# mennowitteveen/PySnpTools

Hardware: AMD Instinct MI355X
Metric: SNPs/sec standardized (500k×1M) + GRM GF/s at 1/2/4/8 GPUs (higher is better)
Workload: dtype f32; 1 GPU; decode+Unit standardize of the 500000 iid x 1000000 SNP matrix (packed BED resident in HBM, SnpGen MAF curve, 1% missing), SNPs split into 1 contiguous shard(s), block 2048 SNPs, f32 F-order block buffer with a 500000-float column pitch; n_iid=500000, n_sid=1000000, n_sid_per_gpu=1000000, block=2048, block_buffer_ld=500000, parallelism=snp-shard x1, process_group=none

## Files before the change

pysnptools_amd/csrc/api.hip:

```cpp
#include <fcntl.h>
#include <immintrin.h>
#include <sys/mman.h>
#include <sys/stat.h>
#include <unistd.h>

#include <algorithm>
#include <atomic>
#include <cmath>
#include <cstdlib>
#include <mutex>
#include <thread>
#include <vector>

#include "snpmi_internal.hpp"

#include <type_traits>

namespace snpmi {

static thread_local std::string g_last_error;
void set_last_error(const std::string& msg) { g_last_error = msg; }

static std::mutex g_dev_mutex;
static std::vector<Device*> g_devices;
// ... 1585 lines not shown

using namespace snpmi;

extern "C" {

const char* snpmi_last_error(void) { return g_last_error.c_str(); }
int snpmi_version(void) { return 1; }

int snpmi_device_count(int* count) {
    return guarded([&] {
        SNPMI_REQUIRE(count != nullptr, SNPMI_E_ARG, "count is NULL");
        *count = num_devices();
        (void)hipGetLastError();
    });
}

int snpmi_set_device(int dev) {
    return guarded([&] {
        SNPMI_REQUIRE(dev >= 0 && dev < num_devices(), SNPMI_E_ARG, "device index out of range");
        g_cur_dev = dev;
        (void)device();
    });
}

int snpmi_get_device(int* dev) {
    return guarded([&] {
        SNPMI_REQUIRE(dev != nullptr, SNPMI_E_ARG, "dev is NULL");
        *dev = g_cur_dev < 0 ? default_device() : g_cur_dev;
    });
}

int snpmi_release_cache(void) {
    return guarded([&] {
        std::lock_guard<std::recursive_mutex> lk(g_call_mutex);
        std::lock_guard<std::mutex> lk2(g_dev_mutex);
        for (Device* d : g_devices)
            if (d) {
                SNPMI_HIP(hipSetDevice(d->id));
                SNPMI_HIP(hipStreamSynchronize(d->stream));
                d->release();
            }
        release_pinned();
    });
}

int snpmi_device_info(int dev, char* name, size_t name_len, uint64_t* total_mem, int* cu_count) {
    return guarded([&] {
        hipDeviceProp_t p;
        SNPMI_HIP(hipGetDeviceProperties(&p, dev));
        if (name && name_len) {
            std::strncpy(name, p.gcnArchName, name_len - 1);
            name[name_len - 1] = 0;
        }
        if (total_mem) *total_mem = p.totalGlobalMem;
        if (cu_count) *cu_count = p.multiProcessorCount;
    });
}

int snpmi_device_ids(int dev, uint8_t* uuid16, int* pci, int* clock_khz) {
    return guarded([&] {
        hipDeviceProp_t p;
        SNPMI_HIP(hipGetDeviceProperties(&p, dev));
        if (uuid16) std::memcpy(uuid16, p.uuid.bytes, 16);
        if (pci) {
            pci[0] = p.pciDomainID;
            pci[1] = p.pciBusID;
            pci[2] = p.pciDeviceID;
        }
        if (clock_khz) *clock_khz = p.clockRate;
    });
}

struct Hook {
    const char* name;
    int* value;
    enum Kind { ANY, BOOL, CLAMP0, RANGE, LIST, READ_ONLY } kind;
    int lo, hi;
    std::vector<int> list;
    const char* what;
};
static const std::vector<Hook>& hooks() {
    static const std::vector<Hook> table = {
        {"decode", &g_variant_decode, Hook::ANY, 0, 0, {}, nullptr},
        {"std", &g_variant_std, Hook::ANY, 0, 0, {}, nullptr},
        {"diag", &g_diag_exact, Hook::BOOL, 0, 0, {}, nullptr},
        {"extract", &g_variant_extract, Hook::ANY, 0, 0, {}, nullptr},
        {"syrk", &g_variant_syrk, Hook::LIST, 0, 0, {0, 5, 20, 36, 71}, "syrk variant: a shipped kernel (0, 5, 20, 36, 71)"},
        {"syrk_split", &g_variant_syrk_split, Hook::ANY, 0, 0, {}, nullptr},
        {"dense_chunk", &g_dense_chunk, Hook::CLAMP0, 0, 0, {}, nullptr},
        {"dense_codes", &g_dense_codes, Hook::ANY, 0, 0, {}, nullptr},
        {"seg", &g_seg_snps, Hook::CLAMP0, 0, 0, {}, nullptr},
        {"gather", &g_gather, Hook::ANY, 0, 0, {}, nullptr},
        {"h2", &g_h2_kernel, Hook::RANGE, 0, 1, {}, "h2 SYRK: 0 = k_syrk_h2, 1 = k_syrk_h2s"},
        {"crt", &g_crt_kernel, Hook::RANGE, 0, 2, {},
         "crt residue SYRK: 0 = k_syrk_i8r, 1 = k_syrk_i8w, 2 = k_syrk_i8w without its read order / wave priorities"},
        {"crt_block", &g_crt_block, Hook::RANGE, 0, 1, {}, "crt moduli: 0 = launch-wide R, 1 = per 256-block"},
        {"f64", &g_f64_mfma, Hook::RANGE, 0, 1, {}, "f64 GRM path: 0 = int8 residues + CRT, 1 = f64 MFMA"},
        {"overlap_groups", &g_last_groups, Hook::READ_ONLY, 0, 0, {}, nullptr},
        {"overlap_calls", &g_last_sum_calls, Hook::READ_ONLY, 0, 0, {}, nullptr},
        {"overlap_sig", &g_last_sum_sig31, Hook::READ_ONLY, 0, 0, {}, nullptr},
    };
    return table;
}
static const Hook& find_hook(const char* name) {
    for (const Hook& h : hooks())
        if (std::strcmp(name, h.name) == 0) return h;
    throw Error(SNPMI_E_ARG, std::string("unknown kernel ") + name);
}

int snpmi_set_kernel_variant(const char* kernel, int variant) {
    return guarded([&] {
        SNPMI_REQUIRE(kernel != nullptr, SNPMI_E_ARG, "kernel name is NULL");
        const Hook& h = find_hook(kernel);
        const bool ok = h.kind == Hook::RANGE  ? variant >= h.lo && variant <= h.hi
                        : h.kind == Hook::LIST ? std::find(h.list.begin(), h.list.end(), variant) != h.list.end()
                                               : h.kind != Hook::READ_ONLY;
        SNPMI_REQUIRE(ok, SNPMI_E_ARG,
                      h.what ? std::string(h.what) + " (got " + std::to_string(variant) + ")"
                             : std::string("unknown kernel ") + kernel);
        *h.value = h.kind == Hook::BOOL ? variant != 0 : h.kind == Hook::CLAMP0 ? std::max(variant, 0) : variant;
    });
}

int snpmi_get_kernel_variant(const char* kernel, int* variant) {
    return guarded([&] {
        SNPMI_REQUIRE(kernel != nullptr && variant != nullptr, SNPMI_E_ARG, "kernel name or output is NULL");
        *variant = *find_hook(kernel).value;
    });
}

int snpmi_bed_check(const char* path, uint64_t n_iid, uint64_t n_sid) {
    return guarded([&] {
        BedMap m;
        open_bed(m, path, n_iid, n_sid);
    });
}

#define SNPMI_BED_READ(SUFFIX, T)                                                                                  \
    int snpmi_bed_read_##SUFFIX(const char* path, uint64_t n_iid, uint64_t n_sid, int count_a1,                  \
                                const uint64_t* iid_idx, uint64_t n_out_iid, const uint64_t* sid_idx,             \
                                uint64_t n_out_sid, int order_c, T* out, int num_threads) {                       \
        return guarded([&] {                                                                                       \
            bed_read_impl<T>(path, n_iid, n_sid, count_a1, iid_idx, n_out_iid, sid_idx, n_out_sid, order_c,       \
                             SNPMI_STD_NONE, 0.0, 0.0, 0, (T*)nullptr, out, num_threads);                         \
        });                                                                                                        \
    }
SNPMI_BED_READ(f32, float)
SNPMI_BED_READ(f64, double)
SNPMI_BED_READ(i8, int8_t)

#define SNPMI_BED_READ_STD(SUFFIX, T)                                                                              \
    int snpmi_bed_read_standardize_##SUFFIX(const char* path, uint64_t n_iid, uint64_t n_sid, int count_a1,      \
                                            const uint64_t* iid_idx, uint64_t n_out_iid, const uint64_t* sid_idx, \
                                            uint64_t n_out_sid, int order_c, int std_kind, double a, double b,    \
                                            int use_stats, T* stats, T* out, int num_threads) {                   \
        return guarded([&] {                                                                                       \
            SNPMI_REQUIRE(std_kind == SNPMI_STD_NONE || stats != nullptr, SNPMI_E_ARG, "stats is NULL");          \
            bed_read_impl<T>(path, n_iid, n_sid, count_a1, iid_idx, n_out_iid, sid_idx, n_out_sid, order_c,       \
                             std_kind, a, b, use_stats, stats, out, num_threads);                                 \
        });                                                                                                        \
    }
SNPMI_BED_READ_STD(f32, float)
SNPMI_BED_READ_STD(f64, double)

#define SNPMI_BED_WRITE(SUFFIX, T)                                                                                 \
    int snpmi_bed_write_##SUFFIX(const char* path, const T* val, uint64_t n_iid, uint64_t n_sid, int order_c,    \
// ... 915 lines not shown
```

pysnptools_amd/csrc/kernels.hip:

```cpp
#include "snpmi_internal.hpp"

namespace snpmi {
namespace {

constexpr int kWave = 64;
constexpr int kBlock = 256;

__device__ __forceinline__ double stats_mean_std(double n, double s1, double s2, double* sd_out) {
    if (n == 0.0) {
        *sd_out = __builtin_nan("");
        return __builtin_nan("");
    }
    double m = s1 / n;
    double var = s2 / n - m * m;
    double sd = sqrt(var);
    if (!(sd > 0.0)) sd = __builtin_inf();
    *sd_out = sd;
    return m;
}

__device__ __forceinline__ double beta_weight(double mean, double a, double b) {
    double maf = mean / 2.0;
    if (maf > 0.5) maf = 1.0 - maf;
    if (!(maf >= 0.0 && maf <= 1.0)) return 0.0;
// ... 67 lines not shown
                count_word(v.w);
            };
            const uint64_t nfull = n / 64;
            constexpr uint64_t step = (uint64_t)W * kWave;
            uint64_t q = (uint64_t)sub * kWave + lane;
            for (; q + (U - 1) * step < nfull; q += U * step) {
                uint4 v[U];
#pragma unroll
                for (int u = 0; u < U; u++) v[u] = col[q + u * step];
#pragma unroll
                for (int u = 0; u < U; u++) count16(v[u]);
            }
            for (; q < nfull; q += step) count16(col[q]);
            if (q == nfull && n % 64) {
                const uint4 v = col[q];
                const uint32_t w4[4] = {v.x, v.y, v.z, v.w};
#pragma unroll
                for (int k = 0; k < 4; k++) {
                    const uint64_t ib = q * 64 + 16 * k;
                    const uint64_t valid_i = n > ib ? min<uint64_t>(n - ib, 16) : 0;
                    const uint32_t mk = valid_i >= 16 ? 0xffffffffu : ((1u << (2 * valid_i)) - 1u);
                    count_word(w4[k] & mk);
                }
            }
            c1 = clo - c3;
            c2 = chi - c3;
        }
        c1 = wave_sum_u32(c1);
        c2 = wave_sum_u32(c2);
        c3 = wave_sum_u32(c3);
        if constexpr (W > 1) {
            if (lane == 0) {
                red[wave][0] = c1;
                red[wave][1] = c2;
                red[wave][2] = c3;
            }
            __syncthreads();
            if (!valid || sub != 0) return;
#pragma unroll
            for (int w = 1; w < W; w++) {
                c1 += red[wave + w][0];
                c2 += red[wave + w][1];
                c3 += red[wave + w][2];
            }
        }
        uint64_t c0 = n - c1 - c2 - c3;
        uint64_t chi = count_a1 ? c0 : c3;
        double nobs = (double)(n - c1);
        mean = stats_mean_std(nobs, (double)(c2 + 2 * chi), (double)(c2 + 4 * chi), &sd);
        if (lane == 0) {
            stats[2 * s] = (T)mean;
            stats[2 * s + 1] = (T)sd;
        }
    }
    if (lane < 4) {
        double w = std_kind == SNPMI_STD_BETA ? beta_weight(mean, a, b) : 0.0;
        bool zero_col = std_kind == SNPMI_STD_BETA && use_stats && __builtin_isinf(sd);
        int v = code_value(lane, count_a1);
        double x;
        if (v < 0 || zero_col) x = 0.0;
        else if (std_kind == SNPMI_STD_BETA) x = ((double)v - mean) * w;
        else x = ((double)v - mean) / sd;
        lut[4 * s + lane] = (T)x;
    }
}

template <typename T>
__device__ __forceinline__ T sel4(T l0, T l1, T l2, T l3, uint32_t c) {
    const bool b0 = (c & 1u) != 0, b1 = (c & 2u) != 0;
    const T lo = b0 ? l1 : l0;
    const T hi = b0 ? l3 : l2;
    return b1 ? hi : lo;
}

typedef float f32x4_t __attribute__((ext_vector_type(4)));
typedef double f64x2_t __attribute__((ext_vector_type(2)));
typedef uint32_t u32x4_t __attribute__((ext_vector_type(4)));

template <typename V>
__device__ __forceinline__ void store_nt(V* p, const V& v) {
    __builtin_nontemporal_store(v, p);
}
template <typename T, int U>
__global__ __launch_bounds__(kBlock) void k_decode_f(const uint8_t* __restrict__ packed, uint64_t pitch, uint64_t n,
                                                     uint64_t m, const T* __restrict__ lut, T* __restrict__ out,
                                                     uint64_t ld) {
    const int lane = threadIdx.x & (kWave - 1);
    const uint64_t chunks = (n + 1023) / 1024;
    const uint64_t total = chunks * m;
    const uint64_t groups = (total + U - 1) / U;
    const uint64_t nwaves = (uint64_t)gridDim.x * (kBlock / kWave);
    const uint64_t lb = (blockIdx.x & 7) * (gridDim.x >> 3) + (blockIdx.x >> 3);
    for (uint64_t gi = lb * (kBlock / kWave) + threadIdx.x / kWave; gi < groups; gi += nwaves) {
        uint32_t w[U];
        uint64_t jv[U], cv[U];
        bool val[U];
#pragma unroll
        for (int u = 0; u < U; u++) {
            const uint64_t it = gi * U + u;
            const uint64_t j = it / chunks, c = it - j * chunks;
            jv[u] = j;
            cv[u] = c;
            val[u] = it < total;
            const bool ok = val[u] && (c * 1024 + 16 * (uint64_t)lane < n);
            w[u] = ok ? reinterpret_cast<const uint32_t*>(packed + j * pitch)[c * 64 + lane] : 0u;
        }
#pragma unroll
        for (int u = 0; u < U; u++) {
            if (!val[u]) continue;
            const uint64_t j = jv[u], i0 = cv[u] * 1024;
            const T l0 = lut[4 * j], l1 = lut[4 * j + 1], l2 = lut[4 * j + 2], l3 = lut[4 * j + 3];
            T* o = out + j * ld + i0;
            if constexpr (sizeof(T) == 4) {
#pragma unroll
                for (int r = 0; r < 4; r++) {
                    const uint32_t src = __shfl(w[u], r * 16 + (lane >> 2), kWave);
                    const uint32_t byte = (src >> (8 * (lane & 3))) & 0xffu;
                    const uint64_t i = i0 + r * 256 + 4 * lane;
                    f32x4_t v;
                    v.x = sel4(l0, l1, l2, l3, byte & 3u);
                    v.y = sel4(l0, l1, l2, l3, (byte >> 2) & 3u);
                    v.z = sel4(l0, l1, l2, l3, (byte >> 4) & 3u);
                    v.w = sel4(l0, l1, l2, l3, byte >> 6);
                    if (i + 4 <= n) {
                        store_nt(reinterpret_cast<f32x4_t*>(o + r * 256 + 4 * lane), v);
                    } else {
                        for (int t = 0; t < 4; t++)
                            if (i + t < n) o[r * 256 + 4 * lane + t] = v[t];
                    }
                }
            } else if constexpr (sizeof(T) == 8) {
#pragma unroll
                for (int r = 0; r < 8; r++) {
                    const uint32_t src = __shfl(w[u], r * 8 + (lane >> 3), kWave);
                    const uint32_t byte = (src >> (8 * ((lane >> 1) & 3))) & 0xffu;
                    const uint32_t sh = 4 * (lane & 1);
                    const uint64_t i = i0 + r * 128 + 2 * lane;
                    f64x2_t v;
                    v.x = sel4(l0, l1, l2, l3, (byte >> sh) & 3u);
                    v.y = sel4(l0, l1, l2, l3, (byte >> (sh + 2)) & 3u);
                    if (i + 2 <= n) {
                        store_nt(reinterpret_cast<f64x2_t*>(o + r * 128 + 2 * lane), v);
                    } else if (i < n) {
                        o[r * 128 + 2 * lane] = v.x;
                    }
                }
            } else {
                const uint32_t lw = (uint32_t)(uint8_t)l0 | ((uint32_t)(uint8_t)l1 << 8) |
                                    ((uint32_t)(uint8_t)l2 << 16) | ((uint32_t)(uint8_t)l3 << 24);
                u32x4_t q;
#pragma unroll
                for (int k = 0; k < 4; k++) {
                    const uint32_t bb = (w[u] >> (8 * k)) & 0xffu;
                    const uint32_t selb = (bb & 3u) | ((bb & 0xCu) << 6) | ((bb & 0x30u) << 12) | ((bb & 0xC0u) << 18);
                    q[k] = __builtin_amdgcn_perm(0u, lw, selb);
                }
                const uint64_t i = i0 + 16 * lane;
                if (i + 16 <= n) {
                    store_nt(reinterpret_cast<u32x4_t*>(o + 16 * lane), q);
                } else if (i < n) {
                    for (uint64_t t = 0; i + t < n; t++)
                        reinterpret_cast<uint8_t*>(o)[16 * lane + t] = (uint8_t)(q[t >> 2] >> (8 * (t & 3)));
                }
            }
        }
    }
}


template <int U>
__global__ __launch_bounds__(kBlock) void k_decode_std_col_f32(const uint8_t* __restrict__ packed, uint64_t pitch,
                                                               uint64_t n, int count_a1, int std_kind, double a,
                                                               double b, int use_stats, float* __restrict__ stats,
                                                               float* __restrict__ lut_out, float* __restrict__ out,
                                                               uint64_t ld) {
    __shared__ uint32_t red[3][kBlock / kWave];
    __shared__ float lutsh[4];
    const int lane = threadIdx.x & (kWave - 1), wave = threadIdx.x / kWave;
    const uint64_t j = blockIdx.x;
    const uint8_t* colp = packed + j * pitch;
    if (std_kind == SNPMI_STD_NONE) {
        if (threadIdx.x < 4) {
            int v = code_value(threadIdx.x, count_a1);
            lutsh[threadIdx.x] = v < 0 ? __builtin_nanf("") : (float)v;
        }
    } else {
        double mean = 0, sd = 0;
        if (!use_stats) {
            const uint4* col = reinterpret_cast<const uint4*>(colp);
            const uint64_t nq = (n + 63) / 64;
            uint32_t c1 = 0, c2 = 0, c3 = 0;
            for (uint64_t q0 = threadIdx.x; q0 < nq; q0 += kBlock * 4) {
                uint4 vv[4];
#pragma unroll
                for (int u = 0; u < 4; u++) {
                    const uint64_t q = q0 + (uint64_t)u * kBlock;
                    vv[u] = q < nq ? col[q] : make_uint4(0, 0, 0, 0);
                }
#pragma unroll
                for (int u = 0; u < 4; u++) {
                    const uint64_t q = q0 + (uint64_t)u * kBlock;
                    uint32_t w4[4] = {vv[u].x, vv[u].y, vv[u].z, vv[u].w};
#pragma unroll
                    for (int k = 0; k < 4; k++) {
                        uint32_t w = w4[k];
                        uint32_t lo = w & 0x55555555u, hi = (w >> 1) & 0x55555555u;
                        const uint64_t ib = q * 64 + 16 * k;
                        if (ib + 16 > n) {
                            const uint64_t valid = n > ib ? n - ib : 0;
                            const uint32_t mk = valid >= 16 ? 0xFFFFFFFFu : (((1u << (2 * valid)) - 1u) & 0x55555555u);
                            lo &= mk;
                            hi &= mk;
                        }
                        c3 += __popc(lo & hi);
                        c2 += __popc(hi & ~lo);
                        c1 += __popc(lo & ~hi);
                    }
                }
            }
            c1 = wave_sum_u32(c1);
            c2 = wave_sum_u32(c2);
            c3 = wave_sum_u32(c3);
            if (lane == 0) {
                red[0][wave] = c1;
                red[1][wave] = c2;
                red[2][wave] = c3;
            }
            __syncthreads();
            if (threadIdx.x == 0) {
                uint64_t t1 = 0, t2 = 0, t3 = 0;
                for (int q = 0; q < kBlock / kWave; q++) {
                    t1 += red[0][q];
                    t2 += red[1][q];
                    t3 += red[2][q];
                }
                const uint64_t c0 = n - t1 - t2 - t3, chi = count_a1 ? c0 : t3;
                mean = stats_mean_std((double)(n - t1), (double)(t2 + 2 * chi), (double)(t2 + 4 * chi), &sd);
                stats[2 * j] = (float)mean;
                stats[2 * j + 1] = (float)sd;
            }
        } else if (threadIdx.x == 0) {
            mean = (double)stats[2 * j];
            sd = (double)stats[2 * j + 1];
        }
        if (threadIdx.x == 0) {
            const double w = std_kind == SNPMI_STD_BETA ? beta_weight(mean, a, b) : 0.0;
            const bool zero_col = std_kind == SNPMI_STD_BETA && use_stats && __builtin_isinf(sd);
            for (int c = 0; c < 4; c++) {
// ... 1377 lines not shown
        c2 = wave_sum_u32(c2);
        c3 = wave_sum_u32(c3);
        if (lane == 0) {
            red[0][wave] = c1;
            red[1][wave] = c2;
            red[2][wave] = c3;
        }
    }
    __syncthreads();
    if (threadIdx.x == 0) {
        if (std_kind == SNPMI_STD_NONE) {
            for (int c = 0; c < 4; c++) {
                const int v = code_value(c, count_a1);
                lutsh[c] = v < 0 ? __builtin_nanf("") : (float)v;
            }
        } else {
            double mean, sd;
            if (count) {
                uint64_t t1 = 0, t2 = 0, t3 = 0;
                for (int q = 0; q < kLdsBlock / kWave; q++) {
                    t1 += red[0][q];
                    t2 += red[1][q];
                    t3 += red[2][q];
                }
                const uint64_t c0 = n - t1 - t2 - t3, chi = count_a1 ? c0 : t3;
                mean = stats_mean_std((double)(n - t1), (double)(t2 + 2 * chi), (double)(t2 + 4 * chi), &sd);
                stats[2 * j] = (float)mean;
                stats[2 * j + 1] = (float)sd;
            } else {
                mean = (double)stats[2 * j];
                sd = (double)stats[2 * j + 1];
            }
            const double w = std_kind == SNPMI_STD_BETA ? beta_weight(mean, a, b) : 0.0;
            const bool zero_col = std_kind == SNPMI_STD_BETA && use_stats && __builtin_isinf(sd);
            for (int c = 0; c < 4; c++) {
                const int v = code_value(c, count_a1);
                double x;
                if (v < 0 || zero_col) x = 0.0;
                else if (std_kind == SNPMI_STD_BETA) x = ((double)v - mean) * w;
                else x = ((double)v - mean) / sd;
                lutsh[c] = (float)x;
            }
        }
        for (int c = 0; c < 4; c++) lut_out[4 * j + c] = lutsh[c];
    }
    __syncthreads();
    const float l0 = lutsh[0], l1 = lutsh[1], l2 = lutsh[2], l3 = lutsh[3];
    const uint32_t* cw = reinterpret_cast<const uint32_t*>(col);
    float* o = out + j * ld;
    const uint64_t chunks = (n + 1023) / 1024;
    for (uint64_t c = wave; c < chunks; c += kLdsBlock / kWave) {
        const uint64_t i0 = c * 1024;
        const uint32_t wv = (i0 + 16 * (uint64_t)lane < n) ? cw[c * 64 + lane] : 0u;
#pragma unroll
        for (int r = 0; r < 4; r++) {
            const uint32_t srcw = __shfl(wv, r * 16 + (lane >> 2), kWave);
            const uint32_t byte = (srcw >> (8 * (lane & 3))) & 0xffu;
            const uint64_t i = i0 + r * 256 + 4 * lane;
            f32x4_t v;
            v.x = sel4(l0, l1, l2, l3, byte & 3u);
            v.y = sel4(l0, l1, l2, l3, (byte >> 2) & 3u);
            v.z = sel4(l0, l1, l2, l3, (byte >> 4) & 3u);
            v.w = sel4(l0, l1, l2, l3, byte >> 6);
            if (i + 4 <= n) {
                store_nt(reinterpret_cast<f32x4_t*>(o + i), v);
            } else {
                for (int t = 0; t < 4; t++)
                    if (i + t < n) o[i + t] = v[t];
            }
        }
    }
}

inline unsigned grid_for(uint64_t work, uint64_t per_block, unsigned cap = 65536) {
    uint64_t g = (work + per_block - 1) / per_block;
    if (g < 1) g = 1;
    if (g > cap) g = cap;
    return (unsigned)g;
}

}

int g_variant_decode = 0;
int g_diag_exact = 1;
int g_variant_std = 0;
int g_variant_extract = 0;

#define SNPMI_LAUNCH_CHECK() SNPMI_HIP(hipGetLastError())

void launch_snp_stats(const uint8_t* packed, uint64_t pitch, uint64_t n, uint64_t m, int count_a1, int std_kind,
                      double a, double b, int use_stats, int dtype, void* stats, void* lut, hipStream_t st) {
    if (m == 0) return;
    const bool wide = n >= 65536 && g_variant_decode != 6;
#define SNPMI_STATS(T, W, kind)                                                                                    \
    k_snp_stats<T, W><<<(unsigned)ceil_div(m, kBlock / kWave / W), kBlock, 0, st>>>(                               \
        packed, pitch, n, m, count_a1, kind, a, b, dtype == SNPMI_DT_I8 ? 0 : use_stats, (T*)stats, (T*)lut)
#define SNPMI_STATS_U(T, W, U, kind)                                                                               \
    k_snp_stats<T, W, U><<<(unsigned)ceil_div(m, kBlock / kWave / W), kBlock, 0, st>>>(                            \
        packed, pitch, n, m, count_a1, kind, a, b, dtype == SNPMI_DT_I8 ? 0 : use_stats, (T*)stats, (T*)lut)
    if (dtype == SNPMI_DT_F32) {
        if (wide && g_variant_decode == 7) SNPMI_STATS_U(float, 4, 4, std_kind);
        else if (wide && g_variant_decode == 9) SNPMI_STATS_U(float, 4, 16, std_kind);
        else if (wide && g_variant_decode == 8) SNPMI_STATS(float, 2, std_kind);
        else if (wide) SNPMI_STATS(float, 4, std_kind);
        else SNPMI_STATS(float, 1, std_kind);
    } else if (dtype == SNPMI_DT_F64) {
        if (wide) SNPMI_STATS(double, 4, std_kind);
        else SNPMI_STATS(double, 1, std_kind);
    } else {
        SNPMI_STATS(int8_t, 1, SNPMI_STD_NONE);
    }
#undef SNPMI_STATS
#undef SNPMI_STATS_U
    SNPMI_LAUNCH_CHECK();
}

void launch_decode(const uint8_t* packed, uint64_t pitch, uint64_t n, uint64_t m, const void* lut, int dtype,
                   int order_c, void* out, uint64_t ld, hipStream_t st) {
    if (m == 0 || n == 0) return;
    if (!order_c) {
        const uint64_t waves = ceil_div(ceil_div(n, 1024) * m, 4);
        const unsigned g = grid_for(waves, kBlock / kWave, 256 * 16 * 8);
        const unsigned g8 = (unsigned)round_up(g, 8);
        if (dtype == SNPMI_DT_F32)
            k_decode_f<float, 4><<<g8, kBlock, 0, st>>>(packed, pitch, n, m, (const float*)lut, (float*)out, ld);
        else if (dtype == SNPMI_DT_F64)
            k_decode_f<double, 4><<<g8, kBlock, 0, st>>>(packed, pitch, n, m, (const double*)lut, (double*)out, ld);
        else
            k_decode_f<int8_t, 4><<<g8, kBlock, 0, st>>>(packed, pitch, n, m, (const int8_t*)lut, (int8_t*)out, ld);
    } else {
        if (dtype != SNPMI_DT_I8 && g_variant_decode != 2 && ld % (16 / dtype_size(dtype)) == 0 &&
            reinterpret_cast<uintptr_t>(out) % 16 == 0 && pitch % 64 == 0) {
            const uint64_t V = 16 / dtype_size(dtype);
            const uint64_t waves = ceil_div(n, 256) * ceil_div(m, 64 * V);
            const unsigned g = grid_for(waves, kBlock / kWave, 256 * 16);
            if (dtype == SNPMI_DT_F32 && g_variant_decode == 3)
                k_decode_c_reg<float, true><<<g, kBlock, 0, st>>>(packed, pitch, n, m, (const float*)lut, (float*)out, ld);
            else if (dtype == SNPMI_DT_F32)
                k_decode_c_reg<float, false><<<g, kBlock, 0, st>>>(packed, pitch, n, m, (const float*)lut, (float*)out,
                                                                   ld);
            else
                k_decode_c_reg<double, false><<<g, kBlock, 0, st>>>(packed, pitch, n, m, (const double*)lut,
                                                                    (double*)out, ld);
            SNPMI_LAUNCH_CHECK();
            return;
        }
        const uint64_t tiles = ceil_div(n, 64) * ceil_div(m, 64);
        const unsigned g = grid_for(tiles, 1, 256 * 8);
        if (dtype == SNPMI_DT_F32)
            k_decode_c<float><<<g, kBlock, 0, st>>>(packed, pitch, n, m, (const float*)lut, (float*)out, ld);
        else if (dtype == SNPMI_DT_F64)
            k_decode_c<double><<<g, kBlock, 0, st>>>(packed, pitch, n, m, (const double*)lut, (double*)out, ld);
        else
            k_decode_c<int8_t><<<g, kBlock, 0, st>>>(packed, pitch, n, m, (const int8_t*)lut, (int8_t*)out, ld);
    }
    SNPMI_LAUNCH_CHECK();
}

void launch_decode_std_fused(const uint8_t* packed, uint64_t pitch, uint64_t n, uint64_t m, int count_a1,
                             int std_kind, double a, double b, int use_stats, void* stats, void* lut, void* out,
                             uint64_t ld, hipStream_t st) {
    if (m == 0 || n == 0) return;
    const uint64_t col_bytes = ceil_div(n, 64) * 16;
    if (g_variant_decode != 1 && col_bytes <= kLdsColMax) {
        SNPMI_HIP(hipFuncSetAttribute((const void*)k_decode_std_lds_f32, hipFuncAttributeMaxDynamicSharedMemorySize,
                                      (int)kLdsColMax));
        k_decode_std_lds_f32<<<(unsigned)m, kLdsBlock, col_bytes, st>>>(packed, pitch, n, count_a1, std_kind, a, b,
                                                                        use_stats, (float*)stats, (float*)lut,
                                                                        (float*)out, ld);
    } else {
        k_decode_std_col_f32<4><<<(unsigned)m, kBlock, 0, st>>>(packed, pitch, n, count_a1, std_kind, a, b, use_stats,
                                                                (float*)stats, (float*)lut, (float*)out, ld);
    }
    SNPMI_LAUNCH_CHECK();
}

uint64_t repack_plan_entries(uint64_t n_out) {
    const uint64_t n = std::max<uint64_t>(n_out, 1);
    return std::max(round_up(n, 16), ceil_div(n, kRepackChunk) * kRepackChunk / 2);
}
uint64_t repack_win_entries(uint64_t n_out) { return 3 * ceil_div(std::max<uint64_t>(n_out, 1), 4096) + 64; }

RepackPlan launch_repack_plan(const uint64_t* idx, uint64_t n_out, uint64_t n_src, uint32_t* plan, uint32_t* win,
                              hipStream_t st) {
    RepackPlan P;
    const uint64_t nq = ceil_div(ceil_div(n_src, 4), 16), n_pad = repack_plan_entries(n_out);
    if (n_out == 0) return P;
    const uint64_t chunk = g_variant_decode == 9 ? 16384 : g_variant_decode == 10 ? 4096 : kRepackChunk;
    const uint64_t nchunks = ceil_div(n_out, chunk);
    if (win != nullptr && nchunks > 1 && g_variant_decode != 8) {
        uint32_t* lohi = win + nchunks;
        std::vector<uint32_t> h(2 * nchunks);
        for (uint64_t c = 0; c < nchunks; c++) h[2 * c] = ~0u, h[2 * c + 1] = 0;
        SNPMI_HIP(hipMemcpyAsync(lohi, h.data(), h.size() * 4, hipMemcpyHostToDevice, st));
        k_repack_window<<<(unsigned)ceil_div(n_out, 2048), 256, 0, st>>>(idx, n_out, chunk, lohi);
        SNPMI_LAUNCH_CHECK();
        SNPMI_HIP(hipMemcpyAsync(h.data(), lohi, h.size() * 4, hipMemcpyDeviceToHost, st));
        SNPMI_HIP(hipStreamSynchronize(st));
        std::vector<uint32_t> lo4(nchunks);
        uint64_t w = 0;
        for (uint64_t c = 0; c < nchunks; c++) {
            lo4[c] = h[2 * c] >> 6;
            w = std::max<uint64_t>(w, (h[2 * c + 1] >> 6) - lo4[c] + 1);
        }
        const uint64_t budget = 40 * 1024 - 16;
        int K = 4 * w * 16 <= budget ? 4 : 2 * w * 16 <= budget ? 2 : w * 16 <= budget ? 1 : 0;
        if (g_variant_decode == 11 && K == 4) K = 2;
        if (K > 0 && 2 * w <= nq) {
            SNPMI_HIP(hipMemcpyAsync(win, lo4.data(), nchunks * 4, hipMemcpyHostToDevice, st));
            if (chunk == kRepackChunk && 4 * w < 4096 && g_variant_decode != 17) {
                const uint64_t n_all = nchunks * kRepackChunk;
                k_repack_plan16<<<grid_for(n_all, kBlock, 4096), kBlock, 0, st>>>(idx, n_out, n_all, w, win,
// ... 429 lines not shown
```

pysnptools_amd/csrc/snpmi_internal.hpp:

```cpp
#pragma once
#include <hip/hip_runtime.h>

#include <cstdint>
#include <cstring>
#include <functional>
#include <stdexcept>
#include <string>
#include <vector>

#include "../../include/snpmi.h"

namespace snpmi {

struct Error : std::runtime_error {
    int code;
    Error(int c, const std::string& m) : std::runtime_error(m), code(c) {}
};

void set_last_error(const std::string& msg);

#define SNPMI_HIP(expr)                                                                     \
    do {                                                                                    \
        hipError_t e_ = (expr);                                                             \
        if (e_ != hipSuccess)                                                               \
            throw ::snpmi::Error(SNPMI_E_HIP, std::string(#expr) + ": " + hipGetErrorString(e_)); \
    } while (0)

#define SNPMI_REQUIRE(cond, code, msg)                 \
    do {                                               \
        if (!(cond)) throw ::snpmi::Error(code, msg);  \
    } while (0)

template <class F>
int guarded(F&& body) {
    try {
        body();
        return SNPMI_OK;
    } catch (const Error& e) {
        set_last_error(e.what());
        return e.code;
    } catch (const std::bad_alloc&) {
        set_last_error("host allocation failed");
        return SNPMI_E_NOMEM;
    } catch (const std::exception& e) {
        set_last_error(e.what());
        return SNPMI_E_ARG;
    }
}

__device__ __forceinline__ uint64_t sgpr_u64(uint64_t v) {
    const uint32_t lo = (uint32_t)__builtin_amdgcn_readfirstlane((int)(uint32_t)v);
    const uint32_t hi = (uint32_t)__builtin_amdgcn_readfirstlane((int)(uint32_t)(v >> 32));
    return ((uint64_t)hi << 32) | (uint64_t)lo;
}
__device__ __forceinline__ void* sgpr_ptr(const void* p) {
    return reinterpret_cast<void*>(sgpr_u64(reinterpret_cast<uint64_t>(p)));
}

constexpr int kTile = 128;
inline uint64_t ceil_div(uint64_t a, uint64_t b) { return (a + b - 1) / b; }
inline uint64_t round_up(uint64_t a, uint64_t b) { return ceil_div(a, b) * b; }
inline uint64_t packed_pitch(uint64_t n_iid) { return round_up(ceil_div(n_iid, 4), 64); }
inline uint64_t n_tiles_1d(uint64_t n) { return ceil_div(n, kTile); }
inline uint64_t n_tiles_upper(uint64_t n) { uint64_t t = n_tiles_1d(n); return t * (t + 1) / 2; }
inline size_t dtype_size(int dt) { return dt == SNPMI_DT_F64 ? 8 : dt == SNPMI_DT_F32 ? 4 : 1; }

constexpr int kPieces = 4;
constexpr uint64_t kPieceBytes = 32ull << 20;

struct Device {
    int id = -1;
    hipStream_t stream = nullptr;
    hipStream_t copy = nullptr;
    hipStream_t aux = nullptr;
    int cu_count = 0;
    enum Slot { S_PACKED, S_PACKED2, S_IDX, S_IDX2, S_LUT, S_STATS, S_OUT, S_TILES, S_K, S_DENSE,
                S_DENSE2, S_RED, S_SESSION, S_PACKED_B, S_ZBLK, S_IDX32, S_LUT3, S_H2, S_OUT_B, S_STATS_B,
                S_WIN, S_DPACK, S_DLUT, S_CRTREC, S_SEG, S_STDFLAG, S_DIAG,
                S_RECT, S_RECT_A, S_RECT_B, S_RECT_IDX_A, S_RECT_IDX_B, S_RECT_PLAN_A, S_RECT_PLAN_B, S_RECT_WIN_A,
                S_RECT_WIN_B, S_RECT_PAIRS, S_NUM };
    void* buf[S_NUM] = {};
    hipEvent_t staged[2] = {};
    hipEvent_t consumed[2] = {};
    hipEvent_t produced[2] = {};
    hipEvent_t bounce[2] = {};
    hipEvent_t fence = nullptr;
    hipEvent_t piece[kPieces] = {};
    uint64_t piece_next = 0;
    size_t cap[S_NUM] = {};
    uint32_t* order_tab[2] = {};
    uint64_t order_nb[2] = {};
    void* part_tab = nullptr;
    uint64_t part_key[3] = {};
    void* get(Slot s, size_t bytes);
    void release();
};

Device& device();
hipStream_t stream();

void* pinned(int slot, size_t bytes);
void release_pinned();

extern int g_variant_decode;
extern int g_variant_std;
extern int g_variant_extract;
extern int g_dense_chunk;
extern int g_h2_kernel;
extern int g_seg_snps;
struct SegCtx {
    uint32_t snps = 0;
    uint32_t nslots = 0;
    uint32_t* flags = nullptr;
    float* scratch = nullptr;
};
constexpr uint32_t kSegSlots = 1024;
constexpr uint64_t kSegSlotFloats = 8 * 32 * 64 * 4;
SegCtx seg_ctx();
const uint32_t* packed_block_order(uint64_t nb);
uint64_t part_unit(uint64_t nb, int world);
void part_layout(uint64_t nb, int rank, int world, std::vector<uint32_t>& tab);
struct PartTables {
    const uint32_t* tab = nullptr;
    const int32_t* dslot = nullptr;
    const int32_t* lslot = nullptr;
};
PartTables part_tables(uint64_t nb, int rank, int world);
void launch_snp_stats(const uint8_t* packed, uint64_t pitch, uint64_t n_iid, uint64_t n_sid, int count_a1,
                      int std_kind, double a, double b, int use_stats, int dtype, void* stats, void* lut,
                      hipStream_t st);
void launch_decode(const uint8_t* packed, uint64_t pitch, uint64_t n_iid, uint64_t n_sid, const void* lut,
                   int dtype, int order_c, void* out, uint64_t ld, hipStream_t st);
void launch_decode_std_fused(const uint8_t* packed, uint64_t pitch, uint64_t n, uint64_t m, int count_a1,
                             int std_kind, double a, double b, int use_stats, void* stats, void* lut, void* out,
                             uint64_t ld, hipStream_t st);
struct RepackPlan {
    const uint32_t* plan = nullptr;
    const uint32_t* win = nullptr;
    int K = 1;
    uint64_t zq = 0;
    uint64_t nchunks = 1;
    uint64_t chunk_words = 0;
    bool lanes = false;
};
uint64_t repack_plan_entries(uint64_t n_out);
uint64_t repack_win_entries(uint64_t n_out);
RepackPlan launch_repack_plan(const uint64_t* idx, uint64_t n_out, uint64_t n_src, uint32_t* plan, uint32_t* win,
                              hipStream_t st);
void launch_repack(const uint8_t* src, uint64_t src_pitch, uint64_t n_src, const uint64_t* idx, const RepackPlan& plan,
                   uint64_t n_out, uint64_t n_sid, uint8_t* dst, uint64_t dst_pitch, hipStream_t st);
void launch_dense_codes(const float* Z, uint64_t ldz, uint64_t n, uint64_t m, uint8_t* packed, uint64_t pitch,
                        float* lut, unsigned int* flag, hipStream_t st);
void launch_dense_standardize(void* val, uint64_t rows, uint64_t cols, uint64_t ld, int order_c, int dtype,
                              int std_kind, double a, double b, int use_stats, void* stats, hipStream_t st);
void launch_subset(const void* in, int in_dt, uint64_t rows, uint64_t cols, uint64_t k, int in_order_c,
                   const uint64_t* ri, uint64_t nr, const uint64_t* ci, uint64_t nc, int out_order_c,
                   void* out, int out_dt, hipStream_t st);
void launch_transpose_to_f(const void* in, uint64_t rows, uint64_t cols, int dtype, void* out, uint64_t ld,
                           hipStream_t st);
void launch_grm_extract_rows(const void* tiles, uint64_t n, int dtype, uint64_t r0, uint64_t nr, double scale,
                             void* out, hipStream_t st);
void launch_grm_extract(const void* tiles, uint64_t n, int dtype, const uint64_t* ri, uint64_t nr,
                        const uint64_t* ci, uint64_t nc, int order_c, double scale, void* out, hipStream_t st);
void launch_grm_trace(const void* tiles, uint64_t n, int dtype, double* trace_dev, hipStream_t st);
void launch_part_extract(const void* blocks, const int32_t* lslot, int dtype, const uint64_t* ri, uint64_t nr,
                         const uint64_t* ci, uint64_t nc, int order_c, double scale, void* out, hipStream_t st);
void launch_part_trace(const void* blocks, const int32_t* dslot, uint64_t n, int dtype, double* trace_dev,
                       hipStream_t st);
extern int g_diag_exact;
void launch_diag_begin(const float* K, uint64_t n, const int32_t* dslot, int accumulate, double* diag, hipStream_t st);
void launch_diag_end(const uint8_t* packed, uint64_t pitch, uint64_t n, uint64_t m, const float* lut, float* K,
                     const int32_t* dslot, double* diag, hipStream_t st);
uint64_t diag_scratch_bytes(uint64_t n, uint64_t m);
void launch_diag_sq(const uint8_t* packed, uint64_t pitch, uint64_t n, uint64_t m, const float* lut, double* diag,
                    hipStream_t st);
void launch_diag_patch(float* K, uint64_t n, uint64_t i0, uint64_t i1, const int32_t* dslot, const double* diag,
                       hipStream_t st);
void rccl_sum_on(void* buf, uint64_t count, int dtype, int root, hipStream_t st);
bool rccl_ready();
void launch_dense_scale(void* p, uint64_t count, int dtype, double scale, hipStream_t st);
void launch_sumsq(const void* p, uint64_t count, int dtype, double* out_dev, hipStream_t st);
void launch_dense_trace(const void* K, uint64_t n, int dtype, double* trace_dev, hipStream_t st);
void launch_copy16(const void* src, void* dst, uint64_t bytes, hipStream_t st);
void launch_synth(uint8_t* packed, uint64_t pitch, uint64_t n_iid, uint64_t sid0, uint64_t n_sid, uint64_t seed,
                  double miss_rate, const double* maf_x_dev, const double* maf_cdf_dev, int n_pts, hipStream_t st);
void launch_encode(const void* val, int dtype, int order_c, uint64_t ld, uint64_t n, uint64_t m, int count_a1,
                   uint8_t* packed, uint64_t pitch, unsigned int* bad_dev, hipStream_t st);
// ... 91 lines not shown
```

Measured before the change: 2.542 million SNPs/s.

## Rewrite F-order decode kernel with double-buffered loads and 32-bit group indexing

Replaces the F-order decode kernel with one that walks whole 4-chunk groups per wave, using 32-bit wave-uniform index stepping in place of 64-bit division per item. Loads for the next group are issued before the current group is stored, so memory reads overlap the stores. Ragged tail chunks are handled in a separate loop. The grid cap is raised and exposed as a tuning hook. The old kernel is kept as a fallback for huge sizes or an unaligned int8 LUT. Whether the decode+standardize benchmark path uses this kernel is unclear, since the standardize path may use a separate fused kernel.

```diff
diff --git a/pysnptools_amd/csrc/api.hip b/pysnptools_amd/csrc/api.hip
--- a/pysnptools_amd/csrc/api.hip
+++ b/pysnptools_amd/csrc/api.hip
@@ -1691,6 +1691,7 @@
 static const std::vector<Hook>& hooks() {
     static const std::vector<Hook> table = {
         {"decode", &g_variant_decode, Hook::ANY, 0, 0, {}, nullptr},
+        {"decode_grid", &g_decode_grid, Hook::CLAMP0, 0, 0, {}, nullptr},
         {"std", &g_variant_std, Hook::ANY, 0, 0, {}, nullptr},
         {"diag", &g_diag_exact, Hook::BOOL, 0, 0, {}, nullptr},
         {"extract", &g_variant_extract, Hook::ANY, 0, 0, {}, nullptr},
diff --git a/pysnptools_amd/csrc/kernels.hip b/pysnptools_amd/csrc/kernels.hip
--- a/pysnptools_amd/csrc/kernels.hip
+++ b/pysnptools_amd/csrc/kernels.hip
@@ -173,9 +173,9 @@
     __builtin_nontemporal_store(v, p);
 }
 template <typename T, int U>
-__global__ __launch_bounds__(kBlock) void k_decode_f(const uint8_t* __restrict__ packed, uint64_t pitch, uint64_t n,
-                                                     uint64_t m, const T* __restrict__ lut, T* __restrict__ out,
-                                                     uint64_t ld) {
+__global__ __launch_bounds__(kBlock) void k_decode_f_drain(const uint8_t* __restrict__ packed, uint64_t pitch,
+                                                           uint64_t n, uint64_t m, const T* __restrict__ lut,
+                                                           T* __restrict__ out, uint64_t ld) {
     const int lane = threadIdx.x & (kWave - 1);
     const uint64_t chunks = (n + 1023) / 1024;
     const uint64_t total = chunks * m;
@@ -255,6 +255,156 @@
                 }
             }
         }
+    }
+}
+
+constexpr uint64_t kDecodeMaxN = 1ull << 34, kDecodeMaxM = 1ull << 29, kDecodeMaxItems = 1ull << 31;
+
+__device__ __forceinline__ void group_advance(uint32_t& j, uint32_t& g, uint32_t dj, uint32_t dg, uint32_t per) {
+    j += dj;
+    g += dg;
+    if (g >= per) {
+        g -= per;
+        j++;
+    }
+    j = __builtin_amdgcn_readfirstlane(j);
+    g = __builtin_amdgcn_readfirstlane(g);
+}
+
+template <typename T, bool FULL>
+__device__ __forceinline__ void decode_item_store(uint32_t w, T l0, T l1, T l2, T l3, T* __restrict__ o, uint64_t i0,
+                                                  uint64_t n, int lane) {
+    if constexpr (sizeof(T) == 4) {
+#pragma unroll
+        for (int r = 0; r < 4; r++) {
+            const uint32_t src = __shfl(w, r * 16 + (lane >> 2), kWave);
+            const uint32_t byte = (src >> (8 * (lane & 3))) & 0xffu;
+            f32x4_t v;
+            v.x = sel4(l0, l1, l2, l3, byte & 3u);
+            v.y = sel4(l0, l1, l2, l3, (byte >> 2) & 3u);
+            v.z = sel4(l0, l1, l2, l3, (byte >> 4) & 3u);
+            v.w = sel4(l0, l1, l2, l3, byte >> 6);
+            const uint64_t i = i0 + r * 256 + 4 * lane;
+            if (FULL || i + 4 <= n) {
+                store_nt(reinterpret_cast<f32x4_t*>(o + r * 256 + 4 * lane), v);
+            } else {
+                for (int t = 0; t < 4; t++)
+                    if (i + t < n) o[r * 256 + 4 * lane + t] = v[t];
+            }
+        }
+    } else if constexpr (sizeof(T) == 8) {
+#pragma unroll
+        for (int r = 0; r < 8; r++) {
+            const uint32_t src = __shfl(w, r * 8 + (lane >> 3), kWave);
+            const uint32_t byte = (src >> (8 * ((lane >> 1) & 3))) & 0xffu;
+            const uint32_t sh = 4 * (lane & 1);
+            f64x2_t v;
+            v.x = sel4(l0, l1, l2, l3, (byte >> sh) & 3u);
+            v.y = sel4(l0, l1, l2, l3, (byte >> (sh + 2)) & 3u);
+            const uint64_t i = i0 + r * 128 + 2 * lane;
+            if (FULL || i + 2 <= n) {
+                store_nt(reinterpret_cast<f64x2_t*>(o + r * 128 + 2 * lane), v);
+            } else if (i < n) {
+                o[r * 128 + 2 * lane] = v.x;
+            }
+        }
+    } else {
+        const uint32_t lw = (uint32_t)(uint8_t)l0 | ((uint32_t)(uint8_t)l1 << 8) | ((uint32_t)(uint8_t)l2 << 16) |
+                            ((uint32_t)(uint8_t)l3 << 24);
+        u32x4_t q;
+#pragma unroll
+        for (int k = 0; k < 4; k++) {
+            const uint32_t bb = (w >> (8 * k)) & 0xffu;
+            const uint32_t selb = (bb & 3u) | ((bb & 0xCu) << 6) | ((bb & 0x30u) << 12) | ((bb & 0xC0u) << 18);
+            q[k] = __builtin_amdgcn_perm(0u, lw, selb);
+        }
+        const uint64_t i = i0 + 16 * lane;
+        if (FULL || i + 16 <= n) {
+            store_nt(reinterpret_cast<u32x4_t*>(o + 16 * lane), q);
+        } else if (i < n) {
+            for (uint64_t t = 0; i + t < n; t++)
+                reinterpret_cast<uint8_t*>(o)[16 * lane + t] = (uint8_t)(q[t >> 2] >> (8 * (t & 3)));
+        }
+    }
+}
+
+template <typename T>
+__device__ __forceinline__ void decode_lut_row(const T* __restrict__ lut, uint32_t j, T (&l)[4]) {
+    if constexpr (sizeof(T) == 1) {
+        const uint32_t x = reinterpret_cast<const uint32_t*>(lut)[j];
+#pragma unroll
+        for (int k = 0; k < 4; k++) l[k] = (T)(x >> (8 * k));
+    } else {
+#pragma unroll
+        for (int k = 0; k < 4; k++) l[k] = lut[4 * (uint64_t)j + k];
+    }
+}
+
+template <int U>
+__device__ __forceinline__ void decode_group_load(const uint8_t* __restrict__ packed, uint64_t pitch, uint32_t m,
+                                                  uint32_t j, uint32_t g, int lane, uint32_t (&w)[U]) {
+    const uint32_t* col = reinterpret_cast<const uint32_t*>(packed + (j < m ? j : m - 1) * pitch) + g * (U * 64);
+#pragma unroll
+    for (int u = 0; u < U; u++)
+        w[u] = __hip_atomic_load(col + u * 64 + lane, __ATOMIC_RELAXED, __HIP_MEMORY_SCOPE_WAVEFRONT);
+}
+
+template <typename T, int U>
+__device__ __forceinline__ void decode_group_store(const uint32_t (&w)[U], const T* __restrict__ lut,
+                                                   T* __restrict__ out, uint64_t ld, uint32_t j, uint32_t g,
+                                                   int lane) {
+    T l[4];
+    decode_lut_row(lut, j, l);
+    T* o = out + j * ld + (uint64_t)g * (U * 1024);
+#pragma unroll
+    for (int u = 0; u < U; u++) decode_item_store<T, true>(w[u], l[0], l[1], l[2], l[3], o + u * 1024, 0, 0, lane);
+}
+
+template <typename T, int U>
+__global__ __launch_bounds__(kBlock) void k_decode_f(const uint8_t* __restrict__ packed, uint64_t pitch, uint64_t n,
+                                                     uint64_t m64, const T* __restrict__ lut, T* __restrict__ out,
+                                                     uint64_t ld) {
+    const int lane = threadIdx.x & (kWave - 1);
+    const uint32_t wave = __builtin_amdgcn_readfirstlane(threadIdx.x / kWave);
+    const uint32_t m = (uint32_t)m64;
+    const uint32_t chunks = (uint32_t)((n + 1023) / 1024);
+    const uint32_t gpc = (uint32_t)(n / 1024) / U;
+    const uint32_t nwaves = gridDim.x * (kBlock / kWave);
+    const uint32_t lb = (blockIdx.x & 7) * (gridDim.x >> 3) + (blockIdx.x >> 3);
+    const uint32_t wid = lb * (kBlock / kWave) + wave;
+    if (gpc > 0 && wid < (uint64_t)gpc * m) {
+        const uint32_t j0 = __builtin_amdgcn_readfirstlane(wid / gpc);
+        const uint32_t dj = __builtin_amdgcn_readfirstlane(nwaves / gpc), dg = nwaves - dj * gpc;
+        uint32_t wa[U], wb[U];
+        uint32_t ja = j0, ga = wid - j0 * gpc, jb = ja, gb = ga;
+        group_advance(jb, gb, dj, dg, gpc);
+        decode_group_load<U>(packed, pitch, m, ja, ga, lane, wa);
+        decode_group_load<U>(packed, pitch, m, jb, gb, lane, wb);
+        decode_group_store<T, U>(wa, lut, out, ld, ja, ga, lane);
+        while (jb < m) {
+            ja = jb, ga = gb;
+            group_advance(ja, ga, dj, dg, gpc);
+            decode_group_load<U>(packed, pitch, m, ja, ga, lane, wa);
+            decode_group_store<T, U>(wb, lut, out, ld, jb, gb, lane);
+            if (ja >= m) break;
+            jb = ja, gb = ga;
+            group_advance(jb, gb, dj, dg, gpc);
+            decode_group_load<U>(packed, pitch, m, jb, gb, lane, wb);
+            decode_group_store<T, U>(wa, lut, out, ld, ja, ga, lane);
+        }
+    }
+    const uint32_t rest = chunks - gpc * U;
+    const uint32_t last_dword = (uint32_t)((n - 1) / 16);
+    for (uint32_t e = wid; e < m * rest; e += nwaves) {
+        const uint32_t j = __builtin_amdgcn_readfirstlane(e / rest), c = gpc * U + (e - j * rest);
+        const uint32_t d = c * 64 + lane;
+        const uint32_t w = reinterpret_cast<const uint32_t*>(packed + j * pitch)[d < last_dword ? d : last_dword];
+        T l[4];
+        decode_lut_row(lut, j, l);
+        const uint64_t i0 = (uint64_t)c * 1024;
+        T* o = out + j * ld + i0;
+        if (i0 + 1024 <= n) decode_item_store<T, true>(w, l[0], l[1], l[2], l[3], o, i0, n, lane);
+        else decode_item_store<T, false>(w, l[0], l[1], l[2], l[3], o, i0, n, lane);
     }
 }
 
@@ -1798,6 +1948,7 @@
 }
 
 int g_variant_decode = 0;
+int g_decode_grid = 0;
 int g_diag_exact = 1;
 int g_variant_std = 0;
 int g_variant_extract = 0;
@@ -1835,15 +1986,26 @@
                    int order_c, void* out, uint64_t ld, hipStream_t st) {
     if (m == 0 || n == 0) return;
     if (!order_c) {
-        const uint64_t waves = ceil_div(ceil_div(n, 1024) * m, 4);
-        const unsigned g = grid_for(waves, kBlock / kWave, 256 * 16 * 8);
+        const uint64_t gpc = n / 1024 / 4;
+        const uint64_t waves = gpc > 0 ? gpc * m : ceil_div(ceil_div(n, 1024) * m, 4);
+        const unsigned cap = g_decode_grid > 0 ? (unsigned)round_up((uint64_t)g_decode_grid, 8) : 1u << 20;
+        const unsigned g = grid_for(waves, kBlock / kWave, cap);
         const unsigned g8 = (unsigned)round_up(g, 8);
-        if (dtype == SNPMI_DT_F32)
-            k_decode_f<float, 4><<<g8, kBlock, 0, st>>>(packed, pitch, n, m, (const float*)lut, (float*)out, ld);
-        else if (dtype == SNPMI_DT_F64)
-            k_decode_f<double, 4><<<g8, kBlock, 0, st>>>(packed, pitch, n, m, (const double*)lut, (double*)out, ld);
-        else
-            k_decode_f<int8_t, 4><<<g8, kBlock, 0, st>>>(packed, pitch, n, m, (const int8_t*)lut, (int8_t*)out, ld);
+        const bool drain = g_variant_decode == 4 ||
+                           (dtype == SNPMI_DT_I8 && reinterpret_cast<uintptr_t>(lut) % 4 != 0) ||
+                           n >= kDecodeMaxN || m >= kDecodeMaxM || ceil_div(n, 1024) * m >= kDecodeMaxItems;
+#define SNPMI_DECODE_F(K)                                                                                          \
+    do {                                                                                                           \
+        if (dtype == SNPMI_DT_F32)                                                                                 \
+            K<float, 4><<<g8, kBlock, 0, st>>>(packed, pitch, n, m, (const float*)lut, (float*)out, ld);           \
+        else if (dtype == SNPMI_DT_F64)                                                                            \
+            K<double, 4><<<g8, kBlock, 0, st>>>(packed, pitch, n, m, (const double*)lut, (double*)out, ld);        \
+        else                                                                                                       \
+            K<int8_t, 4><<<g8, kBlock, 0, st>>>(packed, pitch, n, m, (const int8_t*)lut, (int8_t*)out, ld);        \
+    } while (0)
+        if (drain) SNPMI_DECODE_F(k_decode_f_drain);
+        else SNPMI_DECODE_F(k_decode_f);
+#undef SNPMI_DECODE_F
     } else {
         if (dtype != SNPMI_DT_I8 && g_variant_decode != 2 && ld % (16 / dtype_size(dtype)) == 0 &&
             reinterpret_cast<uintptr_t>(out) % 16 == 0 && pitch % 64 == 0) {
diff --git a/pysnptools_amd/csrc/snpmi_internal.hpp b/pysnptools_amd/csrc/snpmi_internal.hpp
--- a/pysnptools_amd/csrc/snpmi_internal.hpp
+++ b/pysnptools_amd/csrc/snpmi_internal.hpp
@@ -103,6 +103,7 @@
 void release_pinned();
 
 extern int g_variant_decode;
+extern int g_decode_grid;
 extern int g_variant_std;
 extern int g_variant_extract;
 extern int g_dense_chunk;
```

Measured after the change: 2.790 million SNPs/s, median of 6. 9.8% higher.
